# moritzmeister/hops-examples

Measured on AMD Instinct MI355X. Metric: images/sec MNIST CNN + steps/sec Chicago-taxi DNN at 1/2/4/8 MI355X, higher is better.
Workload: dtype bf16; 1 GPU; model=MNIST CNN (experiment.mirrored model, 1394282 params), Adadelta(1.0), global_batch=32, per_gpu_batch=32, parallelism=dp1, engine=PersistentMnistStep, hipgraph=False, steps_per_execution=32, warmup_steps_run=5

## Files before the change

csrc/ops/mnist_persist.hip:

```cpp
#include "common.h"
#include "optim_core.h"

namespace mnistp {

constexpr int B = 32;
constexpr int C1 = 32, C2 = 64, HID = 128, NCLS = 10;
constexpr int PH = 13, NPOS = PH * PH;
constexpr int KIN = NPOS * C2;
constexpr int NCONV = C2 * 128 + C2 + C1 * 4 + C1;
constexpr int OFF_B2 = C2 * 128, OFF_W1 = OFF_B2 + C2, OFF_B1 = OFF_W1 + C1 * 4;
constexpr int SLICE = 52, NSLICE = (NCONV + SLICE - 1) / SLICE;
constexpr int NRED = 19;
constexpr int NHEAD = B;
constexpr int GRID = NPOS + NHEAD;
constexpr int PAY = 272;
constexpr int PAY_DH = 0, PAY_H = 128, PAY_DL = 256, PAY_LOSS = 268, PAY_COR = 269;
constexpr int FL_A = 0, FL_B = 256, FL_C = 512, FL_D = 768, FL_WORDS = 1024;
constexpr int FL_EPOCH = FL_WORDS - 2;
constexpr int D_F32 = OFF_B2 * 2;
constexpr int D_BYTES = D_F32 + (NCONV - OFF_B2) * 4;
constexpr int TGB_N = NHEAD * (HID / 2);
constexpr int TG_WORDS = 2 * 2 * TGB_N;
static_assert(FL_WORDS % 2 == 0 && TGB_N % 256 == 0, "granules are 8-B aligned; every thread owns TGB_N / 256");

// ... 47 lines not shown
typedef unsigned long long __attribute__((address_space(1))) gu64;

struct Args {
  float* master;
  bf16_raw* shadow;
  float* s1;
  float* s2;
  long off[8];
  const unsigned char* xs;
  const long long* ys;
  long nbatch;
  long long* cursor;
  unsigned long long* rng;
  float* step_dev;
  const float* hp_dev;
  float* slabA;
  float* slabB;
  float* slabC;
  float* slabD;
  unsigned* flags;
  unsigned* err;
  float* out;
  unsigned long long* dbg;
  OptHP hp;
  float drop_p, xscale, xshift;
  unsigned salt;
  int nsteps;
  int acquire;
  long long tmo;
  long long tmo0;
  int pollw, stagger;
  int pollw_a, pollw_b, pollw_c, pollw_d;
  int head1w;
  int hand;
  float inv_gb;
  int world, rank;
  int loopback;
  int xfence;
  long long* xstep;
  unsigned char* xbuf[XMAX];
  unsigned* xflag[XMAX];
};

__device__ __forceinline__ __amdgpu_buffer_rsrc_t rsrc(const void* p) {
  return __builtin_amdgcn_make_buffer_rsrc(const_cast<void*>(p), (short)0, 0x7fffffff, 0x00020000);
}
__device__ __forceinline__ void st_sc1(__amdgpu_buffer_rsrc_t r, int byte_off, f32x4 v) {
  __builtin_amdgcn_raw_buffer_store_b128(__builtin_bit_cast(v4i, v), r, byte_off, 0, 16);
}
__device__ __forceinline__ void st_sc1x2(__amdgpu_buffer_rsrc_t r, int byte_off, float x, float y) {
  typedef int v2i __attribute__((ext_vector_type(2)));
  __builtin_amdgcn_raw_buffer_store_b64((v2i){__float_as_int(x), __float_as_int(y)}, r, byte_off, 0, 16);
}
__device__ __forceinline__ f32x4 ld_sc1(__amdgpu_buffer_rsrc_t r, int byte_off) {
  return __builtin_bit_cast(f32x4, __builtin_amdgcn_raw_buffer_load_b128(r, byte_off, 0, 16));
}
__device__ __forceinline__ void drain() { asm volatile("s_waitcnt vmcnt(0)" ::: "memory"); }
__device__ __forceinline__ void flag_store(unsigned* f, unsigned v) {
  __hip_atomic_store((gu32*)f, v, __ATOMIC_RELAXED, __HIP_MEMORY_SCOPE_AGENT);
}
__device__ __forceinline__ unsigned flag_load(const unsigned* f) {
  return __hip_atomic_load((gu32*)f, __ATOMIC_RELAXED, __HIP_MEMORY_SCOPE_AGENT);
}

__device__ __forceinline__ void st_sys(__amdgpu_buffer_rsrc_t r, int byte_off, f32x4 v) {
  __builtin_amdgcn_raw_buffer_store_b128(__builtin_bit_cast(v4i, v), r, byte_off, 0, 17);
}
__device__ __forceinline__ void st_sys1(__amdgpu_buffer_rsrc_t r, int byte_off, float v) {
  __builtin_amdgcn_raw_buffer_store_b32(__float_as_uint(v), r, byte_off, 0, 17);
}
__device__ __forceinline__ f32x4 ld_sys(__amdgpu_buffer_rsrc_t r, int byte_off) {
  return __builtin_bit_cast(f32x4, __builtin_amdgcn_raw_buffer_load_b128(r, byte_off, 0, 17));
}
__device__ __forceinline__ float ld_sys1(__amdgpu_buffer_rsrc_t r, int byte_off) {
  return __uint_as_float(__builtin_amdgcn_raw_buffer_load_b32(r, byte_off, 0, 17));
}
__device__ __forceinline__ void xflag_store(unsigned* f, unsigned v) {
  __hip_atomic_store((gu32*)f, v, __ATOMIC_RELAXED, __HIP_MEMORY_SCOPE_SYSTEM);
}
__device__ __forceinline__ unsigned xflag_load(const unsigned* f) {
  return __hip_atomic_load((gu32*)f, __ATOMIC_RELAXED, __HIP_MEMORY_SCOPE_SYSTEM);
}
__device__ __forceinline__ int xslot(const Args& a, int peer) { return a.loopback ? peer : a.rank; }

__device__ __forceinline__ bool wait_all(const unsigned* flags, int n, unsigned epoch, unsigned* err, unsigned code,
                                      int acquire, int* s_ok, long long tmo, int pollw = 1, int stagger = 0,
                                      int poll1 = 0) {
  if (pollw <= 1) {
    if (threadIdx.x < 64) {
      const int lane = threadIdx.x;
      int good = 1;
      const long long t0 = wall_clock64();
      for (unsigned spins = 0;; ++spins) {
        int ok = 1;
        unsigned e = poll1 ? flag_load(err) : 0u;
        for (int k = lane; k < n; k += 64) ok &= flag_load(flags + k) == epoch;
        if (__all(ok)) break;
        if (!poll1) e = flag_load(err);
        if (__builtin_amdgcn_readfirstlane(e) != 0u) {
          good = 0;
          break;
        }
        if ((spins & 15u) == 15u && wall_clock64() - t0 > tmo) {
          if (lane == 0) atomicCAS(err, 0u, code);
          good = 0;
          break;
        }
        __builtin_amdgcn_s_sleep(1);
      }
      if (acquire && good) __builtin_amdgcn_fence(__ATOMIC_ACQUIRE, "agent");
      drain();
      if (lane == 0) *s_ok = good;
    }
    __syncthreads();
    const int g = *s_ok;
    return g != 0;
  }
  volatile int* gen = s_ok + 1;
  const int wave = threadIdx.x >> 6;
  if (wave < pollw) {
    const int lane = threadIdx.x & 63;
    int good = 1;
    for (int d = 0; d < wave * stagger && __builtin_amdgcn_readfirstlane(*gen) != (int)code; ++d)
      __builtin_amdgcn_s_sleep(1);
    const long long t0 = wall_clock64();
    for (unsigned spins = 0;; ++spins) {
      if (__builtin_amdgcn_readfirstlane(*gen) == (int)code) break;
      int ok = 1;
      unsigned e = poll1 ? flag_load(err) : 0u;
      for (int k = lane; k < n; k += 64) ok &= flag_load(flags + k) == epoch;
      if (__all(ok)) {
        if (lane == 0) {
          s_ok[0] = 1;
          *gen = (int)code;
        }
        break;
      }
      if (!poll1) e = flag_load(err);
      if (__builtin_amdgcn_readfirstlane(e) != 0u) good = 0;
      if ((spins & 15u) == 15u && wall_clock64() - t0 > tmo) {
        if (lane == 0) atomicCAS(err, 0u, code);
        good = 0;
      }
      if (!good) {
        if (lane == 0) {
          s_ok[0] = 0;
          *gen = (int)code;
        }
        break;
      }
      __builtin_amdgcn_s_sleep(1);
    }
    if (acquire) __builtin_amdgcn_fence(__ATOMIC_ACQUIRE, "agent");
    drain();
  }
  __syncthreads();
  const int g = s_ok[0];
  return g != 0;
}

__device__ __forceinline__ bool wait_peers(const Args& a, int base, int stride, unsigned epoch, unsigned code,
                                        int* s_ok) {
  if (threadIdx.x < 64) {
    const int lane = threadIdx.x;
    const unsigned* page = a.xflag[a.rank];
    int good = 1;
    const long long t0 = wall_clock64();
    for (unsigned spins = 0;; ++spins) {
      const bool mine = lane < a.world && lane != a.rank;
      unsigned e = (a.hand & 2) ? flag_load(a.err) : 0u;
      const int ok = !mine || (int)(xflag_load(page + base + lane * stride) - epoch) >= 0;
      if (__all(ok)) break;
      if (!(a.hand & 2)) e = flag_load(a.err);
      if (__builtin_amdgcn_readfirstlane(e) != 0u) {
        good = 0;
        break;
      }
      if ((spins & 15u) == 15u && wall_clock64() - t0 > a.tmo) {
        if (lane == 0) atomicCAS(a.err, 0u, code);
        good = 0;
        break;
      }
      __builtin_amdgcn_s_sleep(1);
    }
    drain();
    if (lane == 0) *s_ok = good;
  }
  __syncthreads();
  const int g = *s_ok;
  return g != 0;
}
__device__ __forceinline__ void raise_peers(const Args& a, int base, int stride, unsigned epoch) {
  if (a.xfence) __builtin_amdgcn_fence(__ATOMIC_RELEASE, "");
  const int r = threadIdx.x & 63;
  if (r < a.world && r != a.rank) xflag_store(a.xflag[r] + base + xslot(a, r) * stride, epoch);
}

__device__ __forceinline__ float adadelta(float w, float g, float& s1, float& s2, const OptHP& h) {
  g = fmaf(h.wd, w, g);
  s1 = fmaf(h.a, s1, (1.f - h.a) * g * g);
  const float delta = g * __builtin_amdgcn_sqrtf(s2 + h.b) * __builtin_amdgcn_rsqf(s1 + h.b);
  s2 = fmaf(h.a, s2, (1.f - h.a) * delta * delta);
  return fmaf(-h.lr, delta, w);
}

__device__ __forceinline__ unsigned ecode(int phase, int s) {
  return 0x80000000u | ((unsigned)phase << 24) | (((unsigned)s & 0xFFFu) << 12) | (blockIdx.x & 0xFFFu);
}

__device__ __forceinline__ bf16_raw f2bf(float f) { return __builtin_bit_cast(bf16_raw, (__bf16)f); }

__device__ __forceinline__ bf16x8 lds8(const bf16_raw* p) { return *(const bf16x8*)p; }
__device__ __forceinline__ bf16x8 lds_tr(const bf16_raw* p1, const bf16_raw* p2) {
  const bf16x4 v1 = __builtin_amdgcn_ds_read_tr16_b64_v4i16((lds_v4_ptr)(p1));
  const bf16x4 v2 = __builtin_amdgcn_ds_read_tr16_b64_v4i16((lds_v4_ptr)(p2));
  return (bf16x8){v1[0], v1[1], v1[2], v1[3], v2[0], v2[1], v2[2], v2[3]};
}
__device__ __forceinline__ f32x4 mfma(bf16x8 a, bf16x8 b, f32x4 c) {
  return __builtin_amdgcn_mfma_f32_16x16x32_bf16(a, b, c, 0, 0, 0);
}

__device__ __forceinline__ long conv_idx(const Args& a, int j) {
  if (j < OFF_B2) return a.off[2] + j;
  if (j < OFF_W1) return a.off[3] + (j - OFF_B2);
  if (j < OFF_B1) return a.off[0] + (j - OFF_W1);
  return a.off[1] + (j - OFF_B1);
}

__device__ __forceinline__ void stamp(const Args& a, int s, int ph) {
  if (a.dbg && threadIdx.x == 0) a.dbg[((long)blockIdx.x * a.nsteps + s) * 16 + ph] = (unsigned long long)wall_clock64();
}

__device__ __forceinline__ void granule_store(unsigned long long* g, unsigned epoch, unsigned value) {
  __hip_atomic_store((gu64*)g, ((unsigned long long)epoch << 32) | value, __ATOMIC_RELAXED, __HIP_MEMORY_SCOPE_AGENT);
}
__device__ __forceinline__ unsigned long long granule_load(const unsigned long long* g) {
  return __hip_atomic_load((gu64*)g, __ATOMIC_RELAXED, __HIP_MEMORY_SCOPE_AGENT);
}
__device__ __forceinline__ bool gate_tags(const unsigned long long* g, int gi, unsigned epoch, int need, unsigned* err,
                                       unsigned code, int* s_ok, long long tmo) {
  if (threadIdx.x < 64) {
    const int lane = threadIdx.x;
    const bool mine = lane < NHEAD;
    int good = 1;
    const long long t0 = wall_clock64();
    for (unsigned spins = 0;; ++spins) {
      const unsigned e = flag_load(err);
      const unsigned long long x = mine ? granule_load(g + lane * (HID / 2) + gi) : 0ull;
      const bool hit = mine && (unsigned)(x >> 32) == epoch;
      if (__popcll(__ballot(hit)) >= need) break;
      if (__builtin_amdgcn_readfirstlane(e) != 0u) {
        good = 0;
        break;
      }
      if ((spins & 15u) == 15u && wall_clock64() - t0 > tmo) {
        if (lane == 0) atomicCAS(err, 0u, code);
        good = 0;
        break;
      }
      __builtin_amdgcn_s_sleep(1);
    }
    if (lane == 0) *s_ok = good;
  }
  __syncthreads();
  const int v = *s_ok;
  return v != 0;
}
template <int N, class F>
__device__ __forceinline__ bool sweep_tags(const unsigned long long* g, int tid, unsigned epoch, unsigned* err,
                                        unsigned code, int* s_fail, long long tmo, F put) {
  unsigned pend = (1u << N) - 1u;
  unsigned long long x[N];
#pragma unroll
  for (int k = 0; k < N; ++k) x[k] = granule_load(g + tid + 256 * k);
  unsigned e = flag_load(err);
  const long long t0 = wall_clock64();
  for (unsigned spins = 0;; ++spins) {
#pragma unroll
    for (int k = 0; k < N; ++k)
      if (((pend >> k) & 1u) && (unsigned)(x[k] >> 32) == epoch) {
        put(tid + 256 * k, (unsigned)x[k]);
        pend &= ~(1u << k);
      }
    if (!__any(pend != 0u)) break;
    bool bad = __builtin_amdgcn_readfirstlane(e) != 0u;
    if (!bad && (spins & 15u) == 15u && wall_clock64() - t0 > tmo) {
      if ((threadIdx.x & 63) == 0) atomicCAS(err, 0u, code);
      bad = true;
    }
    if (bad) {
      if ((threadIdx.x & 63) == 0) *s_fail = 1;
      break;
    }
#pragma unroll
    for (int k = 0; k < N; ++k)
      if ((pend >> k) & 1u) x[k] = granule_load(g + tid + 256 * k);
    e = flag_load(err);
  }
  __syncthreads();
  const int f = *s_fail;
  return f == 0;
}

template <bool DP>
__device__ __forceinline__ void position_wg(const Args& a, unsigned char* smem, int* s_ok, const OptHP& hp,
                                            long long cur0, unsigned long long seed, unsigned long long ctr0,
                                            long long xs0, unsigned long long eb) {
  const int p = blockIdx.x, ph = p / PH, pw = p - ph * PH;
  const int tid = threadIdx.x, lane = tid & 63, w = tid >> 6, fr = lane & 15, fq = lane >> 4;
  const int tq = fr >> 2, tp = fr & 3;
  bf16_raw* W1 = (bf16_raw*)(smem + L_W1);
  bf16_raw* W2 = (bf16_raw*)(smem + L_W2);
  float* CW1 = (float*)(smem + L_CW1);
  float* CB1 = (float*)(smem + L_CB1);
  float* CB2 = (float*)(smem + L_CB2);
  float* XIN = (float*)(smem + L_XIN);
  bf16_raw* C1 = (bf16_raw*)(smem + L_C1);
  bf16_raw* POOL = (bf16_raw*)(smem + L_POOL);
  unsigned char* AM = smem + L_AM;
  bf16_raw* DH = (bf16_raw*)(smem + L_DH);
  bf16_raw* DC2 = (bf16_raw*)(smem + L_DC2);
  float* STG = (float*)(smem + L_STG);
  float* RED = (float*)(smem + L_RED);
  float* SLm = (float*)(smem + L_SL);
  float* SL1 = SLm + 64;
  float* SL2 = SLm + 128;

  float wm[2][4][4], g1[2][4][4], g2[2][4][4];
#pragma unroll
  for (int ii = 0; ii < 2; ++ii)
#pragma unroll
    for (int j = 0; j < 4; ++j)
#pragma unroll
      for (int r = 0; r < 4; ++r) {
        const int n = (2 * w + ii) * 16 + fq * 4 + r, co = j * 16 + fr;
        const long ai = a.off[4] + (long)n * KIN + p * C2 + co;
        wm[ii][j][r] = a.master[ai];
        g1[ii][j][r] = a.s1[ai];
        g2[ii][j][r] = a.s2[ai];
        W1[n * W1S + co] = f2bf(wm[ii][j][r]);
      }
  auto put_conv = [&](int j, float v) {
    if (j < OFF_B2) W2[(j >> 7) * W2S + (j & 127)] = f2bf(v);
    else if (j < OFF_W1) CB2[j - OFF_B2] = v;
    else if (j < OFF_B1) CW1[j - OFF_W1] = v;
    else CB1[j - OFF_B1] = v;
  };
  {
    constexpr int NJ = (NCONV + 255) / 256;
    float cv[NJ];
#pragma unroll
    for (int q = 0; q < NJ; ++q) {
      const int j = tid + 256 * q;
      cv[q] = j < NCONV ? a.master[conv_idx(a, j)] : 0.f;
    }
#pragma unroll
    for (int q = 0; q < NJ; ++q) {
      const int j = tid + 256 * q;
      if (j < NCONV) put_conv(j, cv[q]);
    }
  }
  const bool owner = p < NSLICE;
  if (owner && tid < SLICE) {
    const int e = p * SLICE + tid;
    if (e < NCONV) {
      const long ci = conv_idx(a, e);
      SLm[tid] = a.master[ci];
      SL1[tid] = a.s1[ci];
      SL2[tid] = a.s2[ci];
    }
  }
  const int xb = tid >> 3, xr = (tid >> 1) & 3, xh = tid & 1;
  auto xload = [&](int s) -> unsigned {
    const long bt = (long)((cur0 + s) % a.nbatch);
    const unsigned char* q = a.xs + (bt * B + xb) * 784 + (2 * ph + xr) * 28 + 2 * pw + 2 * xh;
    return *(const unsigned short*)q;
  };
  unsigned xv = xload(0);
  const float P = a.drop_p, inv = P > 0.f ? 1.f / (1.f - P) : 1.f;
  unsigned char* KEEP = smem + L_KEEP;
  auto draw_keep = [&](int s) {
    const unsigned long long ctr = ctr0 + (unsigned long long)s;
    const uint64_t dkey = (uint64_t)seed ^ ((uint64_t)a.salt * 0xD1B54A32D192ED03ull) ^
                          ((uint64_t)ctr * 0x8CB92BA72F3D8DD7ull);
    for (int e = threadIdx.x; e < B * C2; e += 256) {
      const int b = e >> 6, co = e & 63;
      const long gb = (long)a.rank * B + b;
      KEEP[e] = P > 0.f ? (unsigned char)(uniform01(dkey, (uint64_t)((gb * NPOS + p) * C2 + co)) >= P) : 1;
    }
  };
  draw_keep(0);
  __syncthreads();

  for (int s = 0; s < a.nsteps; ++s) {
    const unsigned ep = (unsigned)(eb + (unsigned long long)s + 1ull);
    const int par = s & 1;
    int oz;
    asm volatile("v_mov_b32 %0, 0" : "=v"(oz));
    const int tid = threadIdx.x + oz, lane = tid & 63, w = tid >> 6, fr = lane & 15, fq = lane >> 4;
    const int tq = fr >> 2, tp = fr & 3, xb = tid >> 3, xr = (tid >> 1) & 3, xh = tid & 1;
    stamp(a, s, 0);
    XIN[xb * 16 + xr * 4 + 2 * xh] = (float)(xv & 0xFFu) * a.xscale + a.xshift;
    XIN[xb * 16 + xr * 4 + 2 * xh + 1] = (float)(xv >> 8) * a.xscale + a.xshift;
    __syncthreads();
    {
      const int ci = tid & 31, bg = tid >> 5;
      const float k0 = CW1[ci * 4 + 0], k1 = CW1[ci * 4 + 1], k2 = CW1[ci * 4 + 2], k3 = CW1[ci * 4 + 3];
      const float bias = CB1[ci];
#pragma unroll
      for (int u = 0; u < 4; ++u) {
        const int b = bg * 4 + u;
        const float* xi = XIN + b * 16;
#pragma unroll
        for (int py = 0; py < 3; ++py)
#pragma unroll
          for (int px = 0; px < 3; ++px) {
            float v = bias;
            v = fmaf(xi[py * 4 + px], k0, v);
            v = fmaf(xi[py * 4 + px + 1], k1, v);
            v = fmaf(xi[(py + 1) * 4 + px], k2, v);
            v = fmaf(xi[(py + 1) * 4 + px + 1], k3, v);
            C1[(b * 9 + py * 3 + px) * C1S + ci] = f2bf(fmaxf(v, 0.f));
          }
      }
    }
    __syncthreads();
    {
      f32x4 acc[2][4];
#pragma unroll
      for (int ii = 0; ii < 2; ++ii)
#pragma unroll
        for (int j = 0; j < 4; ++j) acc[ii][j] = (f32x4){0.f, 0.f, 0.f, 0.f};
#pragma unroll
      for (int kk = 0; kk < 4; ++kk) {
        const int di = kk >> 1, dj = kk & 1;
        bf16x8 af[2];
#pragma unroll
        for (int ii = 0; ii < 2; ++ii) {
          const int b = 4 * (2 * w + ii) + (fr >> 2), q = fr & 3;
          const int pos = ((q >> 1) + di) * 3 + (q & 1) + dj;
          af[ii] = lds8(C1 + (b * 9 + pos) * C1S + fq * 8);
        }
#pragma unroll
        for (int j = 0; j < 4; ++j) {
          const bf16x8 bfr = lds8(W2 + (j * 16 + fr) * W2S + kk * 32 + fq * 8);
#pragma unroll
          for (int ii = 0; ii < 2; ++ii) acc[ii][j] = mfma(af[ii], bfr, acc[ii][j]);
        }
      }
#pragma unroll
      for (int ii = 0; ii < 2; ++ii)
#pragma unroll
        for (int j = 0; j < 4; ++j) {
          const int b = 4 * (2 * w + ii) + fq, co = j * 16 + fr;
          const float bias = CB2[co];
          float best = -INFINITY;
          int bi = 0;
#pragma unroll
          for (int r = 0; r < 4; ++r) {
            const float v = bf2f(f2bf(fmaxf(acc[ii][j][r] + bias, 0.f)));
            if (v > best) {
              best = v;
              bi = r;
            }
          }
          if (!(best > 0.f)) bi = 0xFF;
          if (KEEP[b * C2 + co]) {
            best *= inv;
          } else {
            best = 0.f;
            bi = 0xFF;
          }
          POOL[b * PLS + co] = f2bf(best);
          AM[b * C2 + co] = (unsigned char)bi;
        }
    }
    __syncthreads();
    stamp(a, s, 1);
    {
      f32x4 acc[2][2];
#pragma unroll
      for (int i = 0; i < 2; ++i)
#pragma unroll
        for (int jj = 0; jj < 2; ++jj) acc[i][jj] = (f32x4){0.f, 0.f, 0.f, 0.f};
#pragma unroll
      for (int kk = 0; kk < 2; ++kk) {
        bf16x8 af[2], bfr[2];
#pragma unroll
        for (int i = 0; i < 2; ++i) af[i] = lds8(POOL + (i * 16 + fr) * PLS + kk * 32 + fq * 8);
#pragma unroll
        for (int jj = 0; jj < 2; ++jj) bfr[jj] = lds8(W1 + ((2 * w + jj) * 16 + fr) * W1S + kk * 32 + fq * 8);
#pragma unroll
        for (int i = 0; i < 2; ++i)
#pragma unroll
          for (int jj = 0; jj < 2; ++jj) acc[i][jj] = mfma(af[i], bfr[jj], acc[i][jj]);
      }
#pragma unroll
      for (int i = 0; i < 2; ++i)
#pragma unroll
        for (int jj = 0; jj < 2; ++jj)
#pragma unroll
          for (int r = 0; r < 4; ++r) STG[(i * 16 + fq * 4 + r) * HID + (2 * w + jj) * 16 + fr] = acc[i][jj][r];
    }
    __syncthreads();
    {
      const auto R = rsrc(a.slabA + ((long)par * NPOS + p) * (B * HID));
#pragma unroll
      for (int k = 0; k < 4; ++k) {
        const int idx = tid + 256 * k;
        st_sc1(R, idx * 16, *(const f32x4*)(STG + idx * 4));
      }
      drain();
      __syncthreads();
      if (tid == 0) flag_store(a.flags + FL_A + p, ep);
    }
    const unsigned gep = (unsigned)(xs0 + s + 1);
    if constexpr (DP) {
      const int c0 = w * 16 + 4 * tp;
      const f32x4 f = __builtin_bit_cast(f32x4, lds_tr(POOL + (8 * fq + tq) * PLS + c0, POOL + (8 * fq + tq + 4) * PLS + c0));
      for (int r = 0; r < a.world; ++r) {
        if (r == a.rank) continue;
        st_sys(rsrc(a.xbuf[r] + XO_POOL + (par * XMAX + xslot(a, r)) * XS_POOL + (long)p * 4096), (w * 64 + lane) * 16, f);
      }
    }
    if (s + 1 < a.nsteps) xv = xload(s + 1);
    stamp(a, s, 2);
    if (a.hand & 1) {
      const unsigned long long* TB = (const unsigned long long*)(a.flags + FL_WORDS) + par * TGB_N;
      const unsigned code = s ? ecode(2, s) : ecode(12, 0);
      const long long tmo = s ? a.tmo : a.tmo0;
      if (!gate_tags(TB, p & (HID / 2 - 1), ep, (a.hand >> 8), a.err, code, s_ok, tmo)) return;
      if (!sweep_tags<TGB_N / 256>(TB, tid, ep, a.err, code, s_ok + 2, tmo, [&](int idx, unsigned v) {
            *(unsigned*)(DH + (idx >> 6) * DHS + 2 * (idx & 63)) = v;
          }))
        return;
      if constexpr (DP) {
        drain();
        __syncthreads();
        if (tid < 64) raise_peers(a, XF_POOL + p, NPOS, gep);
      }
      stamp(a, s, 3);
    } else {
    if (!wait_all(a.flags + FL_B, NHEAD, ep, a.err, s ? ecode(2, s) : ecode(12, 0), a.acquire, s_ok,
                  s ? a.tmo : a.tmo0, a.pollw_b, a.stagger, (a.hand & 2)))
      return;
    if constexpr (DP) {
      drain();
      __syncthreads();
      if (tid < 64) raise_peers(a, XF_POOL + p, NPOS, gep);
    }
    stamp(a, s, 3);
    {
      const auto R = rsrc(a.slabB + (long)par * NHEAD * PAY);
#pragma unroll
      for (int k = 0; k < 4; ++k) {
        const int idx = tid + 256 * k, b = idx >> 5, n4 = idx & 31;
        const f32x4 v = ld_sc1(R, (b * PAY + PAY_DH + n4 * 4) * 4);
        *(bf16x4*)(DH + b * DHS + n4 * 4) =
            (bf16x4){(short)f2bf(v[0]), (short)f2bf(v[1]), (short)f2bf(v[2]), (short)f2bf(v[3])};
      }
    }
    __syncthreads();
    }
    f32x4 gw[2][4], dp[2];
    {
      if constexpr (!DP) {
#pragma unroll
      for (int ii = 0; ii < 2; ++ii) {
        const int n0 = (2 * w + ii) * 16 + 4 * tp;
        const bf16x8 af = lds_tr(DH + (8 * fq + tq) * DHS + n0, DH + (8 * fq + tq + 4) * DHS + n0);
#pragma unroll
        for (int j = 0; j < 4; ++j) {
          const int c0 = j * 16 + 4 * tp;
          const bf16x8 bfr = lds_tr(POOL + (8 * fq + tq) * PLS + c0, POOL + (8 * fq + tq + 4) * PLS + c0);
          gw[ii][j] = mfma(af, bfr, (f32x4){0.f, 0.f, 0.f, 0.f});
        }
      }
      }
      dp[0] = dp[1] = (f32x4){0.f, 0.f, 0.f, 0.f};
#pragma unroll
      for (int kk = 0; kk < 4; ++kk) {
        const int k1 = kk * 32 + 8 * fq + tq;
        const bf16x8 bfr = lds_tr(W1 + k1 * W1S + w * 16 + 4 * tp, W1 + (k1 + 4) * W1S + w * 16 + 4 * tp);
#pragma unroll
        for (int i = 0; i < 2; ++i) dp[i] = mfma(lds8(DH + (i * 16 + fr) * DHS + kk * 32 + fq * 8), bfr, dp[i]);
      }
    }
    {
      const int co = w * 16 + fr;
      float db = 0.f;
#pragma unroll
      for (int i = 0; i < 2; ++i)
#pragma unroll
        for (int r = 0; r < 4; ++r) {
          const int b = i * 16 + fq * 4 + r;
          const int am = AM[b * C2 + co];
          const bf16_raw gb = am != 0xFF ? f2bf(dp[i][r] * inv) : (bf16_raw)0;
          db += bf2f(gb);
          *(bf16x4*)(DC2 + co * DCS + b * 4) = (bf16x4){(short)(am == 0 ? gb : 0), (short)(am == 1 ? gb : 0),
                                                        (short)(am == 2 ? gb : 0), (short)(am == 3 ? gb : 0)};
        }
      db += __shfl_xor(db, 16, 64);
      db += __shfl_xor(db, 32, 64);
      if (fq == 0) STG[OFF_B2 + co] = db;
    }
    __syncthreads();
    stamp(a, s, 4);
    {
      f32x4 acc[8];
#pragma unroll
      for (int j = 0; j < 8; ++j) acc[j] = (f32x4){0.f, 0.f, 0.f, 0.f};
#pragma unroll
      for (int kk = 0; kk < 4; ++kk) {
        const int k1 = kk * 32 + 8 * fq + tq, b1 = k1 >> 2, q1 = k1 & 3;
        const bf16x8 af = lds8(DC2 + (w * 16 + fr) * DCS + kk * 32 + fq * 8);
#pragma unroll
        for (int j = 0; j < 8; ++j) {
          const int t = j >> 1, ci0 = (j & 1) * 16 + 4 * tp;
          const int pos = ((q1 >> 1) + (t >> 1)) * 3 + (q1 & 1) + (t & 1);
          const bf16x8 bfr = lds_tr(C1 + (b1 * 9 + pos) * C1S + ci0, C1 + ((b1 + 1) * 9 + pos) * C1S + ci0);
          acc[j] = mfma(af, bfr, acc[j]);
        }
      }
#pragma unroll
      for (int j = 0; j < 8; ++j)
#pragma unroll
        for (int r = 0; r < 4; ++r) STG[(w * 16 + fq * 4 + r) * 128 + j * 16 + fr] = acc[j][r];
    }
    __syncthreads();
    {
      const auto R = rsrc(a.slabC + ((long)par * NPOS + p) * NCONV);
#pragma unroll
      for (int k = 0; k < OFF_B2 / 4 / 256; ++k) {
        const int idx = tid + 256 * k;
        st_sc1(R, idx * 16, *(const f32x4*)(STG + idx * 4));
      }
    }
    {
      const int mh = w >> 1, h = w & 1;
      f32x4 acc[4][4];
#pragma unroll
      for (int i = 0; i < 4; ++i)
#pragma unroll
        for (int t = 0; t < 4; ++t) acc[i][t] = (f32x4){0.f, 0.f, 0.f, 0.f};
#pragma unroll
      for (int kk = 0; kk < 2; ++kk) {
        bf16x8 af[4];
        const int k1 = kk * 32 + 8 * fq + tq;
#pragma unroll
        for (int i = 0; i < 4; ++i) {
          const int m0 = (mh * 4 + i) * 16 + 4 * tp;
          af[i] = lds_tr(DC2 + k1 * DCS + m0, DC2 + (k1 + 4) * DCS + m0);
        }
#pragma unroll
        for (int t = 0; t < 4; ++t) {
          const int c0 = (2 * t + h) * 16 + 4 * tp;
          const bf16x8 bfr = lds_tr(W2 + k1 * W2S + c0, W2 + (k1 + 4) * W2S + c0);
#pragma unroll
          for (int i = 0; i < 4; ++i) acc[i][t] = mfma(af[i], bfr, acc[i][t]);
        }
      }
      const int ci = h * 16 + fr;
      float gk[5] = {0.f, 0.f, 0.f, 0.f, 0.f};
#pragma unroll
      for (int i = 0; i < 4; ++i) {
        const int b = 4 * (mh * 4 + i) + fq;
        float d[9];
#pragma unroll
        for (int k = 0; k < 9; ++k) d[k] = 0.f;
#pragma unroll
        for (int t = 0; t < 4; ++t)
#pragma unroll
          for (int q = 0; q < 4; ++q) d[((q >> 1) + (t >> 1)) * 3 + (q & 1) + (t & 1)] += acc[i][t][q];
        const float* xi = XIN + b * 16;
#pragma unroll
        for (int py = 0; py < 3; ++py)
#pragma unroll
          for (int px = 0; px < 3; ++px) {
            const int pos = py * 3 + px;
            const float dd = (short)C1[(b * 9 + pos) * C1S + ci] > 0 ? d[pos] : 0.f;
            gk[0] = fmaf(dd, xi[py * 4 + px], gk[0]);
            gk[1] = fmaf(dd, xi[py * 4 + px + 1], gk[1]);
            gk[2] = fmaf(dd, xi[(py + 1) * 4 + px], gk[2]);
            gk[3] = fmaf(dd, xi[(py + 1) * 4 + px + 1], gk[3]);
            gk[4] += dd;
          }
      }
#pragma unroll
      for (int k = 0; k < 5; ++k) {
        gk[k] += __shfl_xor(gk[k], 16, 64);
        gk[k] += __shfl_xor(gk[k], 32, 64);
      }
      if (fq == 0) {
#pragma unroll
        for (int k = 0; k < 5; ++k) RED[(mh * 32 + ci) * 5 + k] = gk[k];
      }
    }
    __syncthreads();
    if (tid < 32 * 5) {
      const int ci = tid / 5, k = tid - ci * 5;
      const float v = RED[ci * 5 + k] + RED[(32 + ci) * 5 + k];
      if (k < 4) STG[OFF_W1 + ci * 4 + k] = v;
      else STG[OFF_B1 + ci] = v;
    }
    __syncthreads();
    stamp(a, s, 5);
    {
      const auto R = rsrc(a.slabC + ((long)par * NPOS + p) * NCONV);
      const int idx = OFF_B2 / 4 + tid;
      if (idx < NCONV / 4) st_sc1(R, idx * 16, *(const f32x4*)(STG + idx * 4));
      drain();
      __syncthreads();
      if (tid == 0) flag_store(a.flags + FL_C + p, ep);
    }
    stamp(a, s, 6);
    if (owner) {
      if (!wait_all(a.flags + FL_C, NPOS, ep, a.err, ecode(3, s), a.acquire, s_ok, a.tmo, a.pollw_c, a.stagger, (a.hand & 2)))
        return;
      stamp(a, s, 7);
      const int e0 = p * SLICE;
      if (tid < 13 * NRED) {
        const int j = tid % 13, g = tid / 13;
        f32x4 acc = (f32x4){0.f, 0.f, 0.f, 0.f};
        if (e0 + 4 * j < NCONV) {
          const auto R = rsrc(a.slabC + (long)par * NPOS * NCONV);
          constexpr int NK = (NPOS + NRED - 1) / NRED;
          f32x4 v[NK];
#pragma unroll
          for (int k = 0; k < NK; ++k) {
            const int pp = g + NRED * k;
            v[k] = pp < NPOS ? ld_sc1(R, (pp * NCONV + e0 + 4 * j) * 4) : (f32x4){0.f, 0.f, 0.f, 0.f};
          }
#pragma unroll
          for (int k = 0; k < NK; ++k) acc += v[k];
        }
        *(f32x4*)(RED + g * SLICE + 4 * j) = acc;
      }
      __syncthreads();
      const int e = e0 + tid;
      float gs = 0.f;
      if (tid < SLICE) {
        for (int g = 0; g < NRED; ++g) gs += RED[g * SLICE + tid];
      }
      if constexpr (DP) {
        if (tid < 64) {
          if (tid < SLICE) {
            for (int r = 0; r < a.world; ++r) {
              if (r == a.rank) continue;
              st_sys1(rsrc(a.xbuf[r] + XO_CONV + (par * XMAX + xslot(a, r)) * XS_CONV), e * 4, gs);
            }
          }
          drain();
          raise_peers(a, XF_CONV + p, NSLICE, gep);
        }
        if (!wait_peers(a, XF_CONV + p, NSLICE, gep, ecode(6, s), s_ok)) return;
        if (tid < SLICE) {
          const auto X = rsrc(a.xbuf[a.rank] + XO_CONV + (long)par * XMAX * XS_CONV);
          float v[XMAX];
#pragma unroll
          for (int r = 0; r < XMAX; ++r) v[r] = r < a.world && r != a.rank ? ld_sys1(X, (int)(r * XS_CONV) + e * 4) : gs;
          float t = 0.f;
#pragma unroll
          for (int r = 0; r < XMAX; ++r)
            if (r < a.world) t += v[r];
          gs = t;
        }
      }
      if (tid < SLICE) {
        float wn = 0.f;
        if (e < NCONV) {
          SLm[tid] = adadelta(SLm[tid], gs * hp.gscale, SL1[tid], SL2[tid], hp);
          wn = SLm[tid];
        }
        const float wnext = __shfl_down(wn, 1, 64);
        unsigned char* D = (unsigned char*)a.slabD + (long)par * D_BYTES;
        if (e < OFF_B2) {
          if (!(tid & 1))
            __hip_atomic_store((gu32*)(D + e * 2), (unsigned)f2bf(wn) | ((unsigned)f2bf(wnext) << 16),
                               __ATOMIC_RELAXED, __HIP_MEMORY_SCOPE_AGENT);
        } else if (e < NCONV) {
          __hip_atomic_store((gu32*)(D + D_F32 + (e - OFF_B2) * 4), __float_as_uint(wn), __ATOMIC_RELAXED,
                             __HIP_MEMORY_SCOPE_AGENT);
        }
      }
      if (w == 0) {
        drain();
        if (lane == 0) flag_store(a.flags + FL_D + p, ep);
      }
      stamp(a, s, 8);
    }
    if constexpr (DP) {
      if (!wait_peers(a, XF_H, 1, gep, ecode(7, s), s_ok)) return;
      if (!wait_peers(a, XF_POOL + p, NPOS, gep, ecode(8, s), s_ok)) return;
#pragma unroll
      for (int ii = 0; ii < 2; ++ii)
#pragma unroll
        for (int j = 0; j < 4; ++j) gw[ii][j] = (f32x4){0.f, 0.f, 0.f, 0.f};
      const auto XP = rsrc(a.xbuf[a.rank] + XO_POOL + (long)par * XMAX * XS_POOL + (long)p * 4096);
      const auto XD = rsrc(a.xbuf[a.rank] + XO_DHT + (long)par * XMAX * XS_DHT);
      constexpr int PF = 3;
      bf16x8 af[PF][2], bfr[PF][4];
      auto fetch = [&](int r, int b) {
        if (r == a.rank) {
#pragma unroll
          for (int ii = 0; ii < 2; ++ii) {
            const int n0 = (2 * w + ii) * 16 + 4 * tp;
            af[b][ii] = lds_tr(DH + (8 * fq + tq) * DHS + n0, DH + (8 * fq + tq + 4) * DHS + n0);
          }
#pragma unroll
          for (int j = 0; j < 4; ++j) {
            const int c0 = j * 16 + 4 * tp;
            bfr[b][j] = lds_tr(POOL + (8 * fq + tq) * PLS + c0, POOL + (8 * fq + tq + 4) * PLS + c0);
          }
        } else {
#pragma unroll
          for (int ii = 0; ii < 2; ++ii)
            af[b][ii] = __builtin_bit_cast(bf16x8, ld_sys(XD, (int)(r * XS_DHT) + ((2 * w + ii) * 64 + lane) * 16));
#pragma unroll
          for (int j = 0; j < 4; ++j)
            bfr[b][j] = __builtin_bit_cast(bf16x8, ld_sys(XP, (int)(r * XS_POOL) + (j * 64 + lane) * 16));
        }
      };
#pragma unroll
      for (int r = 0; r < PF - 1; ++r)
        if (r < a.world) fetch(r, r);
#pragma unroll
      for (int r = 0; r < XMAX; ++r) {
        if (r < a.world) {
          if (r + PF - 1 < XMAX && r + PF - 1 < a.world) fetch(r + PF - 1, (r + PF - 1) % PF);
#pragma unroll
          for (int ii = 0; ii < 2; ++ii)
#pragma unroll
            for (int j = 0; j < 4; ++j)
              gw[ii][j] += mfma(af[r % PF][ii], bfr[r % PF][j], (f32x4){0.f, 0.f, 0.f, 0.f});
        }
      }
    }
#pragma unroll
    for (int ii = 0; ii < 2; ++ii)
#pragma unroll
      for (int j = 0; j < 4; ++j)
#pragma unroll
        for (int r = 0; r < 4; ++r) {
          wm[ii][j][r] = adadelta(wm[ii][j][r], gw[ii][j][r] * hp.gscale, g1[ii][j][r], g2[ii][j][r], hp);
          W1[((2 * w + ii) * 16 + fq * 4 + r) * W1S + j * 16 + fr] = f2bf(wm[ii][j][r]);
        }
    if (s + 1 < a.nsteps) draw_keep(s + 1);
    stamp(a, s, 9);
    if (!wait_all(a.flags + FL_D, NSLICE, ep, a.err, ecode(4, s), a.acquire, s_ok, a.tmo, a.pollw_d, a.stagger,
                  (a.hand & 2)))
      return;
    stamp(a, s, 10);
    {
      const auto R = rsrc((const unsigned char*)a.slabD + (long)par * D_BYTES);
      constexpr int NB = OFF_B2 * 2 / 16;
      constexpr int NF = (NCONV - OFF_B2) / 4;
      f32x4 dv[NB / 256 + 1];
#pragma unroll
      for (int k = 0; k < NB / 256; ++k) dv[k] = ld_sc1(R, (tid + 256 * k) * 16);
      dv[NB / 256] = tid < NF ? ld_sc1(R, D_F32 + tid * 16) : (f32x4){0.f, 0.f, 0.f, 0.f};
#pragma unroll
      for (int k = 0; k < NB / 256; ++k) {
        const int c = tid + 256 * k;
        *(f32x4*)(W2 + (c >> 4) * W2S + (c & 15) * 8) = dv[k];
      }
      if (tid < NF) {
        const int j = OFF_B2 + tid * 4;
        float* dst = j < OFF_W1 ? CB2 + (j - OFF_B2) : (j < OFF_B1 ? CW1 + (j - OFF_W1) : CB1 + (j - OFF_B1));
        *(f32x4*)dst = dv[NB / 256];
      }
    }
    __syncthreads();
    stamp(a, s, 11);
  }

#pragma unroll
  for (int ii = 0; ii < 2; ++ii)
#pragma unroll
    for (int j = 0; j < 4; ++j)
#pragma unroll
      for (int r = 0; r < 4; ++r) {
        const int n = (2 * w + ii) * 16 + fq * 4 + r, co = j * 16 + fr;
        const long ai = a.off[4] + (long)n * KIN + p * C2 + co;
        a.master[ai] = wm[ii][j][r];
        a.s1[ai] = g1[ii][j][r];
        a.s2[ai] = g2[ii][j][r];
        a.shadow[ai] = f2bf(wm[ii][j][r]);
      }
  if (owner && tid < SLICE) {
    const int e = p * SLICE + tid;
    if (e < NCONV) {
      const long ci = conv_idx(a, e);
      a.master[ci] = SLm[tid];
      a.s1[ci] = SL1[tid];
      a.s2[ci] = SL2[tid];
      a.shadow[ci] = f2bf(SLm[tid]);
    }
  }
  stamp(a, a.nsteps - 1, 14);
  if (p == 0 && tid == 0) {
    if constexpr (DP) a.xstep[0] = xs0 + a.nsteps;
    a.cursor[0] = (cur0 + a.nsteps) % a.nbatch;
    *(unsigned long long*)(a.flags + FL_EPOCH) = eb + (unsigned long long)a.nsteps;
    a.rng[1] = ctr0 + (unsigned long long)a.nsteps;
    if (a.step_dev) a.step_dev[0] += (float)a.nsteps;
  }
}

template <bool DP>
__device__ __forceinline__ void head_wg(const Args& a, unsigned char* smem, int* s_ok, const OptHP& hp,
                                        long long cur0, long long xs0, unsigned long long eb) {
  const int i = blockIdx.x - NPOS;
  const int tid = threadIdx.x, lane = tid & 63;
  float* HW = (float*)(smem + H_W2);
  float* HW1 = HW + NCLS * HID;
  float* HW2 = HW1 + NCLS * HID;
  float* HB2 = (float*)(smem + H_B2);
  float* HB1 = (float*)(smem + H_B1);
  float* RED = (float*)(smem + H_RED);
  float* HH = (float*)(smem + H_H);
  float* LOG = (float*)(smem + H_LOG);
  float* PAYL = (float*)(smem + H_PAY);
  float* ALL = (float*)(smem + H_ALL);
  {
    constexpr int NJ = NCLS * HID / 256;
    float v0[NJ], v1[NJ], v2[NJ];
#pragma unroll
    for (int q = 0; q < NJ; ++q) {
      const long ai = a.off[6] + tid + 256 * q;
      v0[q] = a.master[ai];
      v1[q] = a.s1[ai];
      v2[q] = a.s2[ai];
    }
#pragma unroll
    for (int q = 0; q < NJ; ++q) {
      HW[tid + 256 * q] = v0[q];
      HW1[tid + 256 * q] = v1[q];
      HW2[tid + 256 * q] = v2[q];
    }
  }
  if (tid < NCLS) {
    const long ai = a.off[7] + tid;
    HB2[tid] = a.master[ai];
    HB2[16 + tid] = a.s1[ai];
    HB2[32 + tid] = a.s2[ai];
  }
  if (tid < HID) {
    const long ai = a.off[5] + tid;
    HB1[tid] = a.master[ai];
    HB1[128 + tid] = a.s1[ai];
    HB1[256 + tid] = a.s2[ai];
  }
  if (tid == 0) {
    PAYL[266] = PAYL[267] = PAYL[270] = PAYL[271] = 0.f;
  }
  __syncthreads();

  for (int s = 0; s < a.nsteps; ++s) {
    const unsigned ep = (unsigned)(eb + (unsigned long long)s + 1ull);
    const int par = s & 1;
    const int y = (int)a.ys[((cur0 + s) % a.nbatch) * B + i];
    if (!wait_all(a.flags + FL_A, NPOS, ep, a.err, s ? ecode(1, s) : ecode(12, 0), a.acquire, s_ok,
                  s ? a.tmo : a.tmo0, a.pollw_a, a.stagger, (a.hand & 2)))
      return;
    stamp(a, s, 0);
    {
      const int n4 = tid & 31, g = tid >> 5;
      const auto R = rsrc(a.slabA + (long)par * NPOS * B * HID);
      constexpr int NK = (NPOS + 7) / 8;
      f32x4 v[NK];
#pragma unroll
      for (int k = 0; k < NK; ++k) {
        const int pp = g + 8 * k;
        v[k] = pp < NPOS ? ld_sc1(R, ((pp * B + i) * HID + n4 * 4) * 4) : (f32x4){0.f, 0.f, 0.f, 0.f};
      }
      f32x4 acc = v[0];
#pragma unroll
      for (int k = 1; k < NK; ++k) acc += v[k];
      *(f32x4*)(RED + g * HID + n4 * 4) = acc;
    }
    __syncthreads();
    if (a.head1w) {
      if (tid < 64) {
        const int n0 = 2 * lane;
        float h[2];
#pragma unroll
        for (int u = 0; u < 2; ++u) {
          float v = 0.f;
#pragma unroll
          for (int g = 0; g < 8; ++g) v += RED[g * HID + n0 + u];
          h[u] = fmaxf(v + HB1[n0 + u], 0.f);
        }
        float z[NCLS];
#pragma unroll
        for (int c = 0; c < NCLS; ++c)
          z[c] = wave_sum(fmaf(h[1], HW[c * HID + n0 + 1], h[0] * HW[c * HID + n0])) + HB2[c];
        float m = z[0];
#pragma unroll
        for (int c = 1; c < NCLS; ++c) m = fmaxf(m, z[c]);
        float e[NCLS], se = 0.f, zy = 0.f;
        int am = NCLS;
#pragma unroll
        for (int c = NCLS - 1; c >= 0; --c) {
          e[c] = __expf(z[c] - m);
          if (z[c] == m) am = c;
          if (c == y) zy = z[c];
        }
#pragma unroll
        for (int c = 0; c < NCLS; ++c) se += e[c];
        const float inv_se = 1.f / se;
        float dl[NCLS];
#pragma unroll
        for (int c = 0; c < NCLS; ++c) dl[c] = (e[c] * inv_se - (c == y ? 1.f : 0.f)) * a.inv_gb;
        float dh[2];
#pragma unroll
        for (int u = 0; u < 2; ++u) {
          float d = 0.f;
#pragma unroll
          for (int c = 0; c < NCLS; ++c) d = fmaf(dl[c], HW[c * HID + n0 + u], d);
          dh[u] = h[u] > 0.f ? d : 0.f;
        }
        if (a.hand & 1)
          granule_store((unsigned long long*)(a.flags + FL_WORDS) + (par * NHEAD + i) * (HID / 2) + lane, ep,
                        (unsigned)f2bf(dh[0]) | ((unsigned)f2bf(dh[1]) << 16));
        const auto R = rsrc(a.slabB + ((long)par * NHEAD + i) * PAY);
        st_sc1x2(R, (PAY_DH + n0) * 4, dh[0], dh[1]);
        st_sc1x2(R, (PAY_H + n0) * 4, h[0], h[1]);
        float p0 = 0.f, p1 = 0.f;
#pragma unroll
        for (int c = 0; c < NCLS; c += 2)
          if (lane == c / 2) {
            p0 = dl[c];
            p1 = dl[c + 1];
          }
        if (lane < NCLS / 2) st_sc1x2(R, (PAY_DL + 2 * lane) * 4, p0, p1);
        if (lane == NCLS / 2) st_sc1x2(R, PAY_LOSS * 4, __logf(se) + m - zy, am == y ? 1.f : 0.f);
        drain();
        if (lane == 0) flag_store(a.flags + FL_B + i, ep);
      }
    }
    if (!a.head1w) {
    if (tid < HID) {
      float v = 0.f;
#pragma unroll
      for (int g = 0; g < 8; ++g) v += RED[g * HID + tid];
      HH[tid] = fmaxf(v + HB1[tid], 0.f);
    }
    __syncthreads();
    {
      const int c = tid >> 4, part = tid & 15;
      float v = 0.f;
      if (c < NCLS) {
#pragma unroll
        for (int k = 0; k < 8; ++k) v = fmaf(HH[part + 16 * k], HW[c * HID + part + 16 * k], v);
      }
      v = row_fold<1>(v);
      if (part == 0 && c < NCLS) LOG[c] = v + HB2[c];
    }
    __syncthreads();
    if (tid < 64) {
      const float z = lane < NCLS ? LOG[lane] : -INFINITY;
      const float m = wave_max(z);
      const float e = lane < NCLS ? __expf(z - m) : 0.f;
      const float se = wave_sum(e);
      const unsigned long long hit = __ballot(lane < NCLS && z == m);
      const int am = __ffsll((long long)hit) - 1;
      if (lane < NCLS) PAYL[PAY_DL + lane] = (e / se - (lane == y ? 1.f : 0.f)) * a.inv_gb;
      if (lane == 0) {
        PAYL[PAY_LOSS] = __logf(se) + m - LOG[y];
        PAYL[PAY_COR] = am == y ? 1.f : 0.f;
      }
    }
    __syncthreads();
    if (tid < HID) {
      const float h = HH[tid];
      float d = 0.f;
#pragma unroll
      for (int c = 0; c < NCLS; ++c) d = fmaf(PAYL[PAY_DL + c], HW[c * HID + tid], d);
      PAYL[PAY_DH + tid] = h > 0.f ? d : 0.f;
      PAYL[PAY_H + tid] = h;
    }
    __syncthreads();
    {
      if ((a.hand & 1) && tid < HID / 2)
        granule_store((unsigned long long*)(a.flags + FL_WORDS) + (par * NHEAD + i) * (HID / 2) + tid, ep,
                      (unsigned)f2bf(PAYL[PAY_DH + 2 * tid]) | ((unsigned)f2bf(PAYL[PAY_DH + 2 * tid + 1]) << 16));
      const auto R = rsrc(a.slabB + ((long)par * NHEAD + i) * PAY);
      if (tid < PAY / 4) st_sc1(R, tid * 16, *(const f32x4*)(PAYL + tid * 4));
      drain();
      __syncthreads();
      if (tid == 0) flag_store(a.flags + FL_B + i, ep);
    }
    }
    stamp(a, s, 1);
    if (!wait_all(a.flags + FL_B, NHEAD, ep, a.err, s ? ecode(5, s) : ecode(12, 0), a.acquire, s_ok,
                  s ? a.tmo : a.tmo0, a.pollw, a.stagger, (a.hand & 2)))
      return;
    {
      const auto R = rsrc(a.slabB + (long)par * NHEAD * PAY);
      constexpr int NK = (NHEAD * PAY / 4 + 255) / 256;
      f32x4 v[NK];
#pragma unroll
      for (int k = 0; k < NK; ++k) {
        const int idx = tid + 256 * k;
        v[k] = idx < NHEAD * PAY / 4 ? ld_sc1(R, idx * 16) : (f32x4){0.f, 0.f, 0.f, 0.f};
      }
#pragma unroll
      for (int k = 0; k < NK; ++k) {
        const int idx = tid + 256 * k;
        if (idx < NHEAD * PAY / 4) *(f32x4*)(ALL + idx * 4) = v[k];
      }
    }
    __syncthreads();
    constexpr int NW = NCLS * HID / 256;
    static_assert(NCLS * HID == NW * 256, "fc2 weight split");
    float gl[NW + 2];
#pragma unroll
    for (int k = 0; k < NW; ++k) {
      const int j = tid + 256 * k, c = j / HID, n = j - c * HID;
      float g = 0.f;
#pragma unroll 8
      for (int b = 0; b < B; ++b) g = fmaf(ALL[b * PAY + PAY_DL + c], ALL[b * PAY + PAY_H + n], g);
      gl[k] = g;
    }
    gl[NW] = gl[NW + 1] = 0.f;
    if (tid < HID) {
#pragma unroll 8
      for (int b = 0; b < B; ++b) gl[NW] += ALL[b * PAY + PAY_DH + tid];
    }
    if (tid < NCLS) {
      for (int b = 0; b < B; ++b) gl[NW + 1] += ALL[b * PAY + PAY_DL + tid];
    }
    if constexpr (DP) {
      const unsigned gep = (unsigned)(xs0 + s + 1);
      if (i == 0) {
        bf16_raw* DS = (bf16_raw*)(smem + H_DHS);
        for (int e = tid; e < B * HID; e += 256) DS[(e >> 7) * DHS + (e & 127)] = f2bf(ALL[(e >> 7) * PAY + PAY_DH + (e & 127)]);
        __syncthreads();
        const int w = tid >> 6, fr = lane & 15, fq = lane >> 4, tq = fr >> 2, tp = fr & 3;
        f32x4 fd[2];
#pragma unroll
        for (int ii = 0; ii < 2; ++ii) {
          const int n0 = (2 * w + ii) * 16 + 4 * tp;
          fd[ii] = __builtin_bit_cast(f32x4, lds_tr(DS + (8 * fq + tq) * DHS + n0, DS + (8 * fq + tq + 4) * DHS + n0));
        }
        for (int r = 0; r < a.world; ++r) {
          if (r == a.rank) continue;
          const int sl = xslot(a, r);
          const auto XG = rsrc(a.xbuf[r] + XO_FC2 + (par * XMAX + sl) * XS_FC2);
#pragma unroll
          for (int k = 0; k < NW; ++k) st_sys1(XG, (tid + 256 * k) * 4, gl[k]);
          if (tid < HID) st_sys1(XG, (NCLS * HID + tid) * 4, gl[NW]);
          if (tid < NCLS) st_sys1(XG, (NCLS * HID + HID + tid) * 4, gl[NW + 1]);
          const auto XD = rsrc(a.xbuf[r] + XO_DHT + (par * XMAX + sl) * XS_DHT);
#pragma unroll
          for (int ii = 0; ii < 2; ++ii) st_sys(XD, ((2 * w + ii) * 64 + lane) * 16, fd[ii]);
        }
        drain();
        __syncthreads();
        if (tid < 64) raise_peers(a, XF_H, 1, gep);
      }
      if (!wait_peers(a, XF_H, 1, gep, ecode(9, s), s_ok)) return;
      const auto X = rsrc(a.xbuf[a.rank] + XO_FC2 + (long)par * XMAX * XS_FC2);
      float t[NW + 2];
#pragma unroll
      for (int k = 0; k < NW + 2; ++k) t[k] = 0.f;
      float v[XMAX][NW + 2];
#pragma unroll
      for (int r = 0; r < XMAX; ++r) {
        const bool peer = r < a.world && r != a.rank;
        const int o = (int)(r * XS_FC2);
#pragma unroll
        for (int k = 0; k < NW; ++k) v[r][k] = peer ? ld_sys1(X, o + (tid + 256 * k) * 4) : gl[k];
        v[r][NW] = peer && tid < HID ? ld_sys1(X, o + (NCLS * HID + tid) * 4) : gl[NW];
        v[r][NW + 1] = peer && tid < NCLS ? ld_sys1(X, o + (NCLS * HID + HID + tid) * 4) : gl[NW + 1];
      }
#pragma unroll
      for (int r = 0; r < XMAX; ++r)
        if (r < a.world) {
#pragma unroll
          for (int k = 0; k < NW + 2; ++k) t[k] += v[r][k];
        }
#pragma unroll
      for (int k = 0; k < NW + 2; ++k) gl[k] = t[k];
    }
#pragma unroll
    for (int k = 0; k < NW; ++k) {
      const int j = tid + 256 * k;
      HW[j] = adadelta(HW[j], gl[k] * hp.gscale, HW1[j], HW2[j], hp);
    }
    if (tid < HID) HB1[tid] = adadelta(HB1[tid], gl[NW] * hp.gscale, HB1[128 + tid], HB1[256 + tid], hp);
    if (tid < NCLS) HB2[tid] = adadelta(HB2[tid], gl[NW + 1] * hp.gscale, HB2[16 + tid], HB2[32 + tid], hp);
    if (i == 0 && tid == 255) {
      float l = 0.f, cc = 0.f;
      for (int b = 0; b < B; ++b) {
        l += ALL[b * PAY + PAY_LOSS];
        cc += ALL[b * PAY + PAY_COR];
      }
      a.out[2 * s] = l * (1.f / B);
      a.out[2 * s + 1] = cc;
    }
    __syncthreads();
    stamp(a, s, 2);
  }
  if (i == 0) {
    for (int j = tid; j < NCLS * HID; j += 256) {
      const long ai = a.off[6] + j;
      a.master[ai] = HW[j];
      a.s1[ai] = HW1[j];
      a.s2[ai] = HW2[j];
      a.shadow[ai] = f2bf(HW[j]);
    }
    if (tid < NCLS) {
      const long ai = a.off[7] + tid;
      a.master[ai] = HB2[tid];
      a.s1[ai] = HB2[16 + tid];
      a.s2[ai] = HB2[32 + tid];
      a.shadow[ai] = f2bf(HB2[tid]);
    }
    if (tid < HID) {
      const long ai = a.off[5] + tid;
      a.master[ai] = HB1[tid];
      a.s1[ai] = HB1[128 + tid];
      a.s2[ai] = HB1[256 + tid];
      a.shadow[ai] = f2bf(HB1[tid]);
    }
  }
}

template <bool DP>
__global__ __launch_bounds__(256, 1) void mnist_persist_k(const Args a) {
  extern __shared__ __attribute__((aligned(16))) unsigned char smem[];
  __shared__ int s_ok[3];
  stamp(a, 0, 13);
  if (threadIdx.x == 0) s_ok[0] = s_ok[1] = s_ok[2] = 0;
  const OptHP hp = load_hp(a.hp, a.hp_dev);
  const long long cur0 = a.cursor[0];
  const long long xs0 = DP ? a.xstep[0] : 0;
  const unsigned long long eb = *(const unsigned long long*)(a.flags + FL_EPOCH);
  if (blockIdx.x < NPOS) {
    position_wg<DP>(a, smem, s_ok, hp, cur0, a.rng[0], a.rng[1], xs0, eb);
  } else {
    head_wg<DP>(a, smem, s_ok, hp, cur0, xs0, eb);
  }
}

}

static int g_persist_reload = 0;
extern "C" void hopsx_mnist_persist_reload_knobs() { g_persist_reload = 1; }

extern "C" int hopsx_mnist_persist(const uint64_t* p, int np, const long* iv, int ni, const float* fv, int nf,
                                   hipStream_t st) {
  using namespace mnistp;
  if (np < 18 || ni < 18 || nf < 8) return (int)hipErrorInvalidValue;
  if (iv[11] != B || iv[10] < 1 || iv[8] < 1) return (int)hipErrorInvalidValue;
  const int world = (int)iv[13], rank = (int)iv[14];
  if (world < 1 || world > XMAX || rank < 0 || rank >= world) return (int)hipErrorInvalidValue;
  const bool dp = world > 1;
  if (dp && np < 19 + 2 * world) return (int)hipErrorInvalidValue;
  Args a{};
  a.master = (float*)p[0];
  a.shadow = (bf16_raw*)p[1];
  a.s1 = (float*)p[2];
  a.s2 = (float*)p[3];
  a.xs = (const unsigned char*)p[4];
  a.ys = (const long long*)p[5];
  a.cursor = (long long*)p[6];
  a.rng = (unsigned long long*)p[7];
  a.step_dev = (float*)p[8];
  a.hp_dev = (const float*)p[9];
  a.slabA = (float*)p[10];
  a.slabB = (float*)p[11];
  a.slabC = (float*)p[12];
  a.slabD = (float*)p[13];
  a.flags = (unsigned*)p[14];
  a.err = (unsigned*)p[15];
  a.out = (float*)p[16];
  a.dbg = (unsigned long long*)p[17];
  for (int k = 0; k < 8; ++k) a.off[k] = iv[k];
  a.nbatch = iv[8];
  a.salt = (unsigned)iv[9];
  a.nsteps = (int)iv[10];
  a.acquire = (int)iv[12];
  a.world = world;
  a.rank = rank;
  a.loopback = (int)iv[15];
  a.xfence = (int)iv[17];
  a.tmo = (long long)iv[16] * 100000ll;
  a.tmo0 = a.tmo;
  static int kn_ok = 0, kn_pollw, kn_stagger, kn_a, kn_b, kn_c, kn_d, kn_head1w, kn_memset, kn_coop;
  static int kn_tagged, kn_gate, kn_poll1;
  static long kn_start_ms;
  if (!kn_ok || g_persist_reload) {
    auto pw = [&](const char* name, long dflt) {
      const long v = hopsx_env_int(name, dflt);
      return (int)(v >= 1 && v <= 4 ? v : 1);
    };
    kn_pollw = pw("HOPSX_PERSIST_POLLW", 1);
    kn_stagger = (int)hopsx_env_int("HOPSX_PERSIST_STAGGER", 12);
    kn_a = pw("HOPSX_PERSIST_POLLW_A", kn_pollw);
    kn_b = pw("HOPSX_PERSIST_POLLW_B", kn_pollw);
    kn_c = pw("HOPSX_PERSIST_POLLW_C", 4);
    kn_d = pw("HOPSX_PERSIST_POLLW_D", kn_pollw);
    kn_head1w = (int)hopsx_env_int("HOPSX_PERSIST_HEAD1W", 1);
    kn_memset = (int)hopsx_env_int("HOPSX_PERSIST_MEMSET", 0);
    kn_coop = (int)hopsx_env_int("HOPSX_PERSIST_COOP", 0);
    kn_start_ms = hopsx_env_int("HOPSX_PERSIST_START_MS", 50);
    kn_tagged = hopsx_env_int("HOPSX_PERSIST_TAGGED", 1) != 0;
    const long gt = hopsx_env_int("HOPSX_PERSIST_GATE", NHEAD / 2);
    kn_gate = (int)(gt >= 1 && gt <= NHEAD ? gt : NHEAD / 2);
    kn_poll1 = hopsx_env_int("HOPSX_PERSIST_POLL1", 1) != 0;
    kn_ok = 1;
    g_persist_reload = 0;
  }
  a.pollw = kn_pollw;
  a.stagger = kn_stagger;
  a.pollw_a = kn_a;
  a.pollw_b = kn_b;
  a.pollw_c = kn_c;
  a.pollw_d = kn_d;
  a.head1w = kn_head1w;
  a.hand = kn_tagged | (kn_poll1 << 1) | (kn_gate << 8);
  if (kn_start_ms > 0 && kn_start_ms * 100000ll < a.tmo) a.tmo0 = kn_start_ms * 100000ll;
  a.inv_gb = 1.f / (float)(world * B);
  if (dp) {
    a.xstep = (long long*)p[18];
    for (int r = 0; r < world; ++r) {
      a.xbuf[r] = (unsigned char*)p[19 + r];
      a.xflag[r] = (unsigned*)p[19 + world + r];
      if (!a.xbuf[r] || !a.xflag[r] || ((uint64_t)a.xbuf[r] & 15)) return (int)hipErrorInvalidValue;
    }
  }
  a.drop_p = fv[0];
  a.xscale = fv[1];
  a.xshift = fv[2];
  a.hp = OptHP{fv[3], fv[4], fv[5], fv[6], fv[7], 0.f, 0.f, 0.f};
  static bool attr[2] = {false, false};
  const void* fn = dp ? (const void*)mnist_persist_k<true> : (const void*)mnist_persist_k<false>;
  if (!attr[dp]) {
    const hipError_t e = hipFuncSetAttribute(fn, hipFuncAttributeMaxDynamicSharedMemorySize, LDS_BYTES);
    if (e != hipSuccess) return (int)e;
    attr[dp] = true;
  }
  if (kn_memset) {
    const hipError_t e = hipMemsetAsync(a.flags, 0, FL_WORDS * sizeof(unsigned), st);
    if (e != hipSuccess) return (int)e;
  }
  if (kn_coop) {
    void* kargs[] = {(void*)&a};
    const hipError_t e = hipLaunchCooperativeKernel(fn, dim3(GRID), dim3(256), kargs, LDS_BYTES, st);
    if (e != hipSuccess) {
      (void)hipGetLastError();
      return (int)e;
    }
    return (int)hipSuccess;
  }
  if (dp)
    hipLaunchKernelGGL(mnist_persist_k<true>, dim3(GRID), dim3(256), LDS_BYTES, st, a);
  else
    hipLaunchKernelGGL(mnist_persist_k<false>, dim3(GRID), dim3(256), LDS_BYTES, st, a);
  return (int)hipGetLastError();
}

extern "C" int hopsx_mnist_persist_occupancy(int dp) {
  using namespace mnistp;
  const void* fn = dp ? (const void*)mnist_persist_k<true> : (const void*)mnist_persist_k<false>;
  if (hipFuncSetAttribute(fn, hipFuncAttributeMaxDynamicSharedMemorySize, LDS_BYTES) != hipSuccess) return -1;
  int n = 0;
  if (hipOccupancyMaxActiveBlocksPerMultiprocessor(&n, fn, 256, LDS_BYTES) != hipSuccess) return -1;
  return n;
}

extern "C" void hopsx_mnist_persist_geom(long* g) {
  using namespace mnistp;
  g[0] = B;
  g[1] = NPOS;
  g[2] = NHEAD;
  g[3] = GRID;
  g[4] = NCONV;
  g[5] = NSLICE;
  g[6] = SLICE;
  g[7] = PAY;
  g[8] = FL_WORDS;
  g[9] = LDS_BYTES;
  g[10] = D_BYTES;
  g[11] = X_BYTES;
  g[12] = XF_WORDS;
  g[13] = XMAX;
  g[14] = XO_POOL;
  g[15] = XS_POOL;
  g[16] = XO_DHT;
  g[17] = XS_DHT;
  g[18] = XO_FC2;
  g[19] = XS_FC2;
  g[20] = XO_CONV;
  g[21] = XS_CONV;
  g[22] = TG_WORDS;
}
```

Measured before the change: 1.382 million images/sec.

## Gather conv-gradient rows progressively as each producer flag arrives

```diff
diff --git a/csrc/ops/mnist_persist.hip b/csrc/ops/mnist_persist.hip
--- a/csrc/ops/mnist_persist.hip
+++ b/csrc/ops/mnist_persist.hip
@@ -373,6 +373,33 @@
   return f == 0;
 }
 
+template <int NK, class L>
+__device__ __forceinline__ void gather_rows(const unsigned* flag, bool mine, int shift, unsigned pend, unsigned epoch,
+                                            unsigned* err, unsigned code, int* s_fail, long long tmo, L load) {
+  const long long t0 = wall_clock64();
+  for (unsigned spins = 0;; ++spins) {
+    const unsigned e = flag_load(err);
+    const unsigned f = mine ? flag_load(flag) : 0u;
+    const unsigned long long here = __ballot(mine && f == epoch);
+    const unsigned now = pend & (unsigned)(here >> shift);
+#pragma unroll
+    for (int k = 0; k < NK; ++k)
+      if ((now >> k) & 1u) load(k);
+    pend &= ~now;
+    if (!__any(pend != 0u)) break;
+    bool bad = __builtin_amdgcn_readfirstlane(e) != 0u;
+    if (!bad && (spins & 15u) == 15u && wall_clock64() - t0 > tmo) {
+      if ((threadIdx.x & 63) == 0) atomicCAS(err, 0u, code);
+      bad = true;
+    }
+    if (bad) {
+      if ((threadIdx.x & 63) == 0) *s_fail = 1;
+      break;
+    }
+    __builtin_amdgcn_s_sleep(1);
+  }
+}
+
 template <bool DP>
 __device__ __forceinline__ void position_wg(const Args& a, unsigned char* smem, int* s_ok, const OptHP& hp,
                                             long long cur0, unsigned long long seed, unsigned long long ctr0,
@@ -786,10 +813,36 @@
     }
     stamp(a, s, 6);
     if (owner) {
+      const int e0 = p * SLICE;
+      constexpr int NKC = (NPOS + NRED - 1) / NRED;
+      static_assert(6 * NKC <= 64, "the flags of a wave's groups (64 threads span at most 6 groups of 13): one per lane");
+      if ((a.hand & 8) && !a.acquire) {
+        const int j = tid % 13, g = tid / 13;
+        const bool act = g < NRED && e0 + 4 * j < NCONV;
+        const int g0 = (w * 64) / 13, g1 = (w * 64 + 63) / 13;
+        const int lg = g0 + lane / NKC, lp = lg + NRED * (lane % NKC);
+        const bool mine = lane < 6 * NKC && lg <= g1 && lg < NRED && lp < NPOS;
+        const auto R = rsrc(a.slabC + (long)par * NPOS * NCONV);
+        f32x4 v[NKC];
+#pragma unroll
+        for (int k = 0; k < NKC; ++k) v[k] = (f32x4){0.f, 0.f, 0.f, 0.f};
+        const unsigned pend = !act ? 0u : (g + NRED * (NKC - 1) < NPOS ? (1u << NKC) - 1u : (1u << (NKC - 1)) - 1u);
+        gather_rows<NKC>(a.flags + FL_C + lp, mine, act ? (g - g0) * NKC : 0, pend, ep, a.err, ecode(3, s), s_ok + 2,
+                         a.tmo, [&](int k) { v[k] = ld_sc1(R, ((g + NRED * k) * NCONV + e0 + 4 * j) * 4); });
+        stamp(a, s, 7);
+        if (g < NRED) {
+          f32x4 acc = (f32x4){0.f, 0.f, 0.f, 0.f};
+#pragma unroll
+          for (int k = 0; k < NKC; ++k) acc += v[k];
+          *(f32x4*)(RED + g * SLICE + 4 * j) = acc;
+        }
+        __syncthreads();
+        const int f = s_ok[2];
+        if (f) return;
+      } else {
       if (!wait_all(a.flags + FL_C, NPOS, ep, a.err, ecode(3, s), a.acquire, s_ok, a.tmo, a.pollw_c, a.stagger, (a.hand & 2)))
         return;
       stamp(a, s, 7);
-      const int e0 = p * SLICE;
       if (tid < 13 * NRED) {
         const int j = tid % 13, g = tid / 13;
         f32x4 acc = (f32x4){0.f, 0.f, 0.f, 0.f};
@@ -808,6 +861,7 @@
         *(f32x4*)(RED + g * SLICE + 4 * j) = acc;
       }
       __syncthreads();
+      }
       const int e = e0 + tid;
       float gs = 0.f;
       if (tid < SLICE) {
@@ -1361,7 +1415,7 @@
   a.tmo = (long long)iv[16] * 100000ll;
   a.tmo0 = a.tmo;
   static int kn_ok = 0, kn_pollw, kn_stagger, kn_a, kn_b, kn_c, kn_d, kn_head1w, kn_memset, kn_coop;
-  static int kn_tagged, kn_gate, kn_poll1;
+  static int kn_tagged, kn_gate, kn_poll1, kn_prog;
   static long kn_start_ms;
   if (!kn_ok || g_persist_reload) {
     auto pw = [&](const char* name, long dflt) {
@@ -1382,6 +1436,7 @@
     const long gt = hopsx_env_int("HOPSX_PERSIST_GATE", NHEAD / 2);
     kn_gate = (int)(gt >= 1 && gt <= NHEAD ? gt : NHEAD / 2);
     kn_poll1 = hopsx_env_int("HOPSX_PERSIST_POLL1", 1) != 0;
+    kn_prog = (int)(hopsx_env_int("HOPSX_PERSIST_PROG", 3) & 2);
     kn_ok = 1;
     g_persist_reload = 0;
   }
@@ -1392,7 +1447,7 @@
   a.pollw_c = kn_c;
   a.pollw_d = kn_d;
   a.head1w = kn_head1w;
-  a.hand = kn_tagged | (kn_poll1 << 1) | (kn_gate << 8);
+  a.hand = kn_tagged | (kn_poll1 << 1) | (kn_prog << 2) | (kn_gate << 8);
   if (kn_start_ms > 0 && kn_start_ms * 100000ll < a.tmo) a.tmo0 = kn_start_ms * 100000ll;
   a.inv_gb = 1.f / (float)(world * B);
   if (dp) {
```

Measured after the change: 1.410 million images/sec (median of 6 runs). +2.0%, better.
